# tspooner/rl_markets

Measured on NVIDIA H100. Metric: env steps/sec (batched LOBs), higher is better.
Workload: dtype f64

## Files before the change

rl_markets_b200/csrc/rlm_env.cuh:

```cuda
#pragma once
#include <cuda_runtime.h>
#include <math.h>
#include "rlm_types.h"

__constant__ DevParams P;

#define LLMIN ((long long)0x8000000000000000ull)
#ifdef RLM_ROLL_LEVELS
#define LEVEL_UNROLL _Pragma("unroll 1")
#else
#define LEVEL_UNROLL _Pragma("unroll")
#endif

__device__ __forceinline__ double pkey(double p) { return rint(p * 10000.0); }

__device__ __forceinline__ long long d2ll_x86(double d) {
  if (!(d >= -9223372036854775808.0 && d < 9223372036854775808.0)) return LLMIN;
  return (long long)d;
}

static_assert((RLM_MAX_BANDS & (RLM_MAX_BANDS - 1)) == 0, "the band search halves RLM_MAX_BANDS");
__device__ __noinline__ int to_ticks(double price, int* err, int* band_hint = nullptr) {
  const VenueD& V = P.venue;
  if (price < V.px[0]) { *err |= ERR_TICK_RANGE; return 0; }
// ... 271 lines not shown
}
__device__ __forceinline__ double win_back(const EnvHdr& e, const double* ring, int w) {
  int i = (e.w_count[w] == P.win_size[w]) ? e.w_head[w] : 0;
  return ring[P.win_off[w] + i];
}
__device__ __forceinline__ double win_std(const EnvHdr& e, int w) {
  double v = e.w_s[w] / (double)((unsigned long long)((long long)e.w_count[w] - 1));
  return v > 0 ? sqrt(v) : 0.0;
}

__device__ __noinline__ double get_reward(const EnvHdr& e) {
  double r = 0.0;
  long long ap = e.position < 0 ? -e.position : e.position;
  int abs_pos = (int)ap;
  switch (P.reward_measure) {
    case RLM_REWARD_NONE: break;
    case RLM_REWARD_PNL: r = e.pnl_step; break;
    case RLM_REWARD_PNL_DAMPED: r = e.pnl_step - (double)P.damping * fmax(0.0, e.momentum_pnl_step); break;
    case RLM_REWARD_SPREAD: r = e.pnl_step / e.w_mean[W_SPREAD]; break;
    case RLM_REWARD_NORMED:
      if (!(e.w_count[W_PNLUP] == P.win_size[W_PNLUP] && e.w_count[W_PNLDN] == P.win_size[W_PNLDN])) r = 0.0;
      else {
        double u = e.w_mean[W_PNLUP], d = e.w_mean[W_PNLDN];
        double su = win_std(e, W_PNLUP), sd = win_std(e, W_PNLDN);
        double numer = (u * sd - d * su), denom = (su + sd);
        if (isnan(numer) || isinf(numer)) numer = 0.0;
        if (isnan(denom) || isinf(denom)) denom = 0.0;
        r = (fabs(denom) < 1e-5) ? numer : (numer / denom);
      }
      break;
    case RLM_REWARD_LOVOL: r = (double)e.lo_vol_step; break;
    case RLM_REWARD_MM_LINEAR: r = (double)(-P.pos_weight * (float)abs_pos); r += (double)P.pnl_weight * e.pnl_step; break;
    case RLM_REWARD_MM_EXP:
      r = -pow(1.0 - exp((double)(P.pos_weight * (float)abs_pos)), 2.0); r += (double)P.pnl_weight * e.pnl_step; break;
    case RLM_REWARD_MM_DIV:
      if (e.pnl_step > 0) r = e.pnl_step / fmax(1.0, (double)abs_pos);
      else r = e.pnl_step;
      break;
  }
  return r * 100.0;
}

__device__ __noinline__ void clear_inventory(EnvHdr& e) {
  long long size = -e.position;
  Fill f; f.volume = 0; f.proxy = 0.0; f.value = 0.0;
  double mip = m_midprice(e);
  if (size > 0) f = side_walk<true>(e.side[0], mip, size);
  else if (size < 0) f = side_walk<false>(e.side[1], mip, size);
  e.position += f.volume;
  e.pnl_step += f.proxy;
  e.lo_vol_step += (int)(f.volume < 0 ? -f.volume : f.volume);
  e.ep_pnl += f.value;
  if (f.volume > 0) e.market_buys++;
  else if (f.volume < 0) e.market_sells++;
}

__device__ __noinline__ void place_orders(EnvHdr& e, int al, int bl) {
  e.ask_level = al; e.bid_level = bl;
  if (P.l2p_book) {
    e.ask_quote = to_price(to_ticks(e.side[0].px[0], &e.err, &e.tk_band) + al, &e.err);
    e.bid_quote = to_price(to_ticks(e.side[1].px[0], &e.err, &e.tk_band) - bl, &e.err);
  } else {
    double tp = e.tp_val, half_spd = fmax(0.0, e.w_mean[W_SPREAD] / 2.0);
    e.ask_quote = to_price(to_ticks(tp + (double)al * half_spd, &e.err, &e.tk_band), &e.err);
    e.bid_quote = to_price(to_ticks(tp - (double)bl * half_spd, &e.err, &e.tk_band), &e.err);
  }
  side_replace_order(e.side[0], e.ask_quote, P.order_size, &e.err);
  side_replace_order(e.side[1], e.bid_quote, P.order_size, &e.err);
}

__device__ __noinline__ void do_action(EnvHdr& e, int action) {
  int al, bl;
  switch (action) {
    case 0: al = 1; bl = 1; break;
    case 1: clear_inventory(e); al = e.ask_level; bl = e.bid_level; break;
    case 2: al = 2; bl = 2; break;
    case 3: al = 3; bl = 3; break;
    case 4: al = 0; bl = 2; break;
    case 5: al = 2; bl = 0; break;
    case 6: al = 1; bl = 4; break;
    case 7: al = 4; bl = 1; break;
    case 8: al = 5; bl = 5; break;
    default: return;
  }
  place_orders(e, al, bl);
}

__device__ __noinline__ void update_stats(EnvHdr& e) {
  e.ts_total++;
  bool has_ask = e.side[0].ord.live, has_bid = e.side[1].ord.live;
  if (has_ask) e.ts_ask++;
  if (has_bid) e.ts_bid++;
  if (has_ask && has_bid) e.ts_both++;
  if (e.position != 0) e.ts_pos++;
  if (e.position > 0) e.ts_long++;
  else if (e.position < 0) e.ts_short++;
}

__device__ __noinline__ void update_book_profiles(EnvHdr& e, const rlm_tick_msg& m) {
  e.last_date = e.date;
  e.date = m.date;
  e.time_ms = m.time_ms;
  side_apply_changes(e.side[0], m.ask_px, m.ask_vol, m, &e.err);
  side_apply_changes(e.side[1], m.bid_px, m.bid_vol, m, &e.err);
  if (e.side[0].has_last && e.side[1].has_last && !(pkey(e.side[0].last_px[0]) == 0.0) && !(pkey(e.side[1].last_px[0]) == 0.0)) {
    double mp = m_midprice(e);
    bool ok = (m_spread(e) >= 0.0) && (mp > 0.0) && (fabs(mp - m_last_midprice(e)) < mp);
    if (!ok) e.err |= ERR_INVALID_STATE;
  }
}

__device__ __noinline__ void next_state_tail(EnvHdr& e, const Fill& au, const Fill& bu, double* pushv) {
  Fill as = adverse_selection(e);
  e.pnl_step += au.proxy + bu.proxy + as.proxy;
  long long asabs = as.volume < 0 ? -as.volume : as.volume;
  e.lo_vol_step += (int)(bu.volume - au.volume + asabs);
  e.ep_pnl += au.value + bu.value + as.value;
  e.position += bu.volume + au.volume + as.volume;
  check_orders(e);
  double mid = m_midprice(e);
  long long mpt;
  if (mid == e.tk_px && mid > 0.0) mpt = e.tk_ticks;
  else { const int t = to_ticks(mid, &e.err, &e.tk_band); mpt = t; e.tk_px = mid; e.tk_ticks = t; }
  double mpm = mid - m_last_midprice(e), sp = m_spread(e);
  pushv[W_MID] = (double)mpt;
  pushv[W_VLT] = (double)mpt;
  pushv[W_VNUM] = e.side[0].obs_value + e.side[1].obs_value;
  pushv[W_VDEN] = (double)(e.side[0].obs_volume + e.side[1].obs_volume);
  pushv[W_SPREAD] = fmax(0.0, sp);
  pushv[W_TP] = P.tp_is_micro ? m_microprice(e) : mid;
  pushv[W_ASKTX] = (double)e.side[0].obs_volume;
  pushv[W_BIDTX] = (double)e.side[1].obs_volume;
  e.ewma_up = (P.ewma_alpha * fmax(0.0, mpm)) + ((1 - P.ewma_alpha) * e.ewma_up);
  e.ewma_dn = (P.ewma_alpha * fabs(fmin(0.0, mpm))) + ((1 - P.ewma_alpha) * e.ewma_dn);
  e.n_ticks++;
}

__device__ __forceinline__ void check_valid_state(EnvHdr& e) {
  if (e.side[0].has_last && e.side[1].has_last && !(pkey(e.side[0].last_px[0]) == 0.0) && !(pkey(e.side[1].last_px[0]) == 0.0)) {
    double mp = m_midprice(e);
    bool ok = (m_spread(e) >= 0.0) && (mp > 0.0) && (fabs(mp - m_last_midprice(e)) < mp);
    if (!ok) e.err |= ERR_INVALID_STATE;
  }
}

__device__ __noinline__ void next_state_scalar(EnvHdr& e, const rlm_tick_msg& m, double* pushv) {
  double mp = m_midprice(e);
  Fill au = side_apply_transactions<true>(e.side[0], m, mp, true);
  Fill bu = side_apply_transactions<false>(e.side[1], m, mp, true);
  update_book_profiles(e, m);
  next_state_tail(e, au, bu, pushv);
}

__device__ __noinline__ void next_state_warp(EnvHdr& e, const rlm_tick_msg& m, double* pushv, Fill* fills, int lane) {
  int* serr = (int*)(fills + 2);
  if (lane < 2) {
    const double mp = m_midprice(e);
    serr[lane] = 0;
    fills[lane] = (lane == 0) ? side_apply_transactions<true>(e.side[0], m, mp, true)
                              : side_apply_transactions<false>(e.side[1], m, mp, true);
  }
  __syncwarp();
  if (lane < 2) side_apply_changes(e.side[lane], lane == 0 ? m.ask_px : m.bid_px, lane == 0 ? m.ask_vol : m.bid_vol, m, &serr[lane]);
  __syncwarp();
  if (lane == 0) {
    e.last_date = e.date; e.date = m.date; e.time_ms = m.time_ms;
    e.err |= serr[0] | serr[1];
    check_valid_state(e);
    next_state_tail(e, fills[0], fills[1], pushv);
  }
}

__device__ __forceinline__ bool needs_multi(const EnvHdr& e, const rlm_tick_msg& m) { return (m.flags & 3) != 0 || e.tick_open != 0 || e.txn != 0; }
__device__ __forceinline__ void tick_tx_append(EnvHdr& e, const rlm_tick_msg& m) {
  for (int i = 0; i < m.n_tx && i < RLM_N_TX_MAX; ++i) {
    if (e.txn >= RLM_TX_CAP) { e.err |= ERR_BAD_PRICE; break; }
    e.tx_px[e.txn] = m.tx_px[i]; e.tx_vol[e.txn] = m.tx_vol[i]; e.txn++;
  }
}
__device__ __noinline__ bool update_book_profiles_multi(EnvHdr& e, const rlm_tick_msg& m, bool with_tx) {
  if (m.flags & RLM_TICK_TX_MORE) { if (with_tx && !e.tick_open) tick_tx_append(e, m); return false; }
  if (!e.tick_open) {
    if (with_tx) tick_tx_append(e, m); else e.txn = 0;
    side_stash(e.side[0]);
    side_stash(e.side[1]);
  }
  e.last_date = e.date;
  e.date = m.date;
  e.time_ms = m.time_ms;
  side_apply_row(e.side[0], m.ask_px, m.ask_vol, e.tx_px, e.tx_vol, e.txn, &e.err);
  side_apply_row(e.side[1], m.bid_px, m.bid_vol, e.tx_px, e.tx_vol, e.txn, &e.err);
  if (m.flags & RLM_TICK_PARTIAL) { e.tick_open = 1; return false; }
  e.tick_open = 0;
  e.txn = 0;
  return true;
}
__device__ __noinline__ bool next_state_multi(EnvHdr& e, const rlm_tick_msg& m, double* pushv) {
  if (m.flags & RLM_TICK_TX_MORE) { if (!e.tick_open) tick_tx_append(e, m); return false; }
  if (!e.tick_open) {
    tick_tx_append(e, m);
    const double mp = m_midprice(e);
    const Fill au = side_apply_transactions_n<true>(e.side[0], e.tx_px, e.tx_vol, e.txn, mp);
    const Fill bu = side_apply_transactions_n<false>(e.side[1], e.tx_px, e.tx_vol, e.txn, mp);
    e.tick_au.volume = au.volume; e.tick_au.proxy = au.proxy; e.tick_au.value = au.value;
    e.tick_bu.volume = bu.volume; e.tick_bu.proxy = bu.proxy; e.tick_bu.value = bu.value;
    side_stash(e.side[0]);
    side_stash(e.side[1]);
  }
  e.last_date = e.date;
  e.date = m.date;
  e.time_ms = m.time_ms;
  side_apply_row(e.side[0], m.ask_px, m.ask_vol, e.tx_px, e.tx_vol, e.txn, &e.err);
  side_apply_row(e.side[1], m.bid_px, m.bid_vol, e.tx_px, e.tx_vol, e.txn, &e.err);
  if (m.flags & RLM_TICK_PARTIAL) { e.tick_open = 1; return false; }
  e.tick_open = 0;
  e.txn = 0;
  check_valid_state(e);
  Fill au, bu;
  au.volume = e.tick_au.volume; au.proxy = e.tick_au.proxy; au.value = e.tick_au.value;
  bu.volume = e.tick_bu.volume; bu.proxy = e.tick_bu.proxy; bu.value = e.tick_bu.value;
  next_state_tail(e, au, bu, pushv);
  return true;
}

__device__ __forceinline__ double ulb_ref(double val, double lb, double ub) {
  const double m = (ub < val) ? ub : val;
  return (m < lb) ? lb : m;
}

__device__ __forceinline__ bool var_tick_args(const EnvHdr& e, const double* ring, int v, double& x0, double& x1) {
  switch (v) {
    case RLM_VAR_SPD: x0 = e.side[0].px[0]; x1 = e.side[1].px[0]; return true;
    case RLM_VAR_MPM: x0 = win_front(e, ring, W_MID); x1 = win_back(e, ring, W_MID); return true;
    case RLM_VAR_A_DIST: if (!e.side[0].ord.live) return false; x0 = e.side[0].ord.price; x1 = e.side[0].px[0]; return true;
    case RLM_VAR_B_DIST: if (!e.side[1].ord.live) return false; x0 = e.side[1].px[0]; x1 = e.side[1].ord.price; return true;
  }
  return false;
}
__device__ __forceinline__ double var_from_ticks(int v, int t0, int t1) {
  switch (v) {
    case RLM_VAR_SPD: return ulb_ref((double)(t0 - t1), 0.0, 20.0);
    case RLM_VAR_MPM: return ulb_ref((double)(t0 - t1), -10.0, 10.0);
  }
  return (double)t0 - (double)t1;
}

__device__ __noinline__ double get_variable(EnvHdr& e, const double* ring, int v) {
  switch (v) {
    case RLM_VAR_POS: return (double)e.position / (double)P.order_size;
    case RLM_VAR_SPD: {
      double d = (double)(to_ticks(e.side[0].px[0], &e.err, &e.tk_band) - to_ticks(e.side[1].px[0], &e.err, &e.tk_band));
      return ulb_ref(d, 0.0, 20.0);
    }
    case RLM_VAR_MPM: {
      double d = (double)(to_ticks(win_front(e, ring, W_MID), &e.err, &e.tk_band) - to_ticks(win_back(e, ring, W_MID), &e.err, &e.tk_band));
      return ulb_ref(d, -10.0, 10.0);
    }
    case RLM_VAR_IMB: {
      double v_a = (double)e.side[0].total_vol, v_b = (double)e.side[1].total_vol;
      return ((v_a + v_b) > 0 ? 5.0 * (v_b - v_a) / (v_b + v_a) : 0.0);
    }
    case RLM_VAR_SVL: {
      double q_a = e.w_sum[W_ASKTX], q_b = e.w_sum[W_BIDTX];
      return ((q_a + q_b) > 0 ? 5.0 * (q_b - q_a) / (q_a + q_b) : 0.0);
    }
    case RLM_VAR_VOL: return ulb_ref(5.0 * win_std(e, W_VLT), 0.0, 10.0);
    case RLM_VAR_RSI: {
      double u = e.ewma_up, d = e.ewma_dn;
      return (u + d) != 0.0 ? 5.0 * (u - d) / (u + d) : 0.0;
    }
    case RLM_VAR_VWAP: {
      double d = e.w_sum[W_VNUM] / e.w_sum[W_VDEN];
      return ulb_ref(d / e.w_mean[W_SPREAD], -10.0, 10.0);
    }
    case RLM_VAR_A_DIST:
      if (e.side[0].ord.live) return ((double)to_ticks(e.side[0].ord.price, &e.err, &e.tk_band) - (double)to_ticks(e.side[0].px[0], &e.err, &e.tk_band));
      else return -100.0;
    case RLM_VAR_A_QUEUE:
      if (e.side[0].ord.live) {
        float qp = (float)e.side[0].ord.q_head / fmaxf(1.0f, (float)e.side[0].ord.initial_queue);
        return 10.0 * (double)(long long)qp;
      } else return -1.0;
    case RLM_VAR_B_DIST:
      if (e.side[1].ord.live) return ((double)to_ticks(e.side[1].px[0], &e.err, &e.tk_band) - (double)to_ticks(e.side[1].ord.price, &e.err, &e.tk_band));
      else return -100.0;
    case RLM_VAR_B_QUEUE:
      if (e.side[1].ord.live) {
        float qp = (float)e.side[1].ord.q_head / fmaxf(1.0f, (float)e.side[1].ord.initial_queue);
        return 10.0 * (double)(long long)qp;
      } else return -1.0;
    case RLM_VAR_LAST_ACTION: return (double)e.last_action;
  }
  return 0.0;
}
```

rl_markets_b200/csrc/rlm_kernels.cu:

```cuda
#include <cuda_runtime.h>
#include <stdint.h>
#define RLM_TABLE_QUAL static __device__ const
#include "rlm_flow_tables.h"
#include "rlm_rndseq.h"
#include "rlm_agent.cuh"
#include <cstdio>
#include "rlm_kernels.h"
#define RLM_ENVT_CARVEOUT_DEFAULT 30
#define RLM_SMEM_CARVEOUT 88

#define SCR_Q 0
#define SCR_SS (SCR_Q + 8 * 2 * RLM_MAX_ACTIONS)
#define SCR_IDX (SCR_SS + 4 * SS_SLOTS)
#define SCR_VBUF (SCR_IDX + 4 * 3 * RLM_MAX_ACTIONS * 32)
#define AG_BYTES ((sizeof(AgentD) + 15) & ~(size_t)15)
size_t rlm_scratch_bytes(int is_double) {
  return ((size_t)SCR_VBUF + (size_t)(is_double ? 2 : 1) * RLM_MAX_ACTIONS * VROW * 8 + 15) & ~(size_t)15;
}
size_t rlm_agent_smem_bytes(int warps_per_cta, int scratch_bytes) {
  return (size_t)warps_per_cta * (AG_BYTES + (size_t)scratch_bytes);
}

#define PDL_PROLOGUE() do { asm volatile("griddepcontrol.launch_dependents;" ::: "memory"); asm volatile("griddepcontrol.wait;" ::: "memory"); } while (0)
static bool g_use_pdl = false;
void rlm_set_pdl(int on) { g_use_pdl = on != 0; }
template <typename... KArgs, typename... Args>
static cudaError_t launch_pdl(void (*kernel)(KArgs...), int grid, int block, size_t smem, cudaStream_t st, Args... args) {
  cudaLaunchConfig_t cfg = {};
  cfg.gridDim = dim3(grid); cfg.blockDim = dim3(block); cfg.dynamicSmemBytes = smem; cfg.stream = st;
  cudaLaunchAttribute at[1];
  at[0].id = cudaLaunchAttributeProgrammaticStreamSerialization;
  at[0].val.programmaticStreamSerializationAllowed = g_use_pdl ? 1 : 0;
  cfg.attrs = at; cfg.numAttrs = 1;
  return cudaLaunchKernelEx(&cfg, kernel, args...);
}

#ifdef RLM_TIMING
__device__ unsigned long long g_klog[256][8][2][2];
__device__ __forceinline__ unsigned long long gtime() { unsigned long long t; asm volatile("mov.u64 %0, %%globaltimer;" : "=l"(t)); return t; }
#define KLOG_BEGIN(kind) do { if (threadIdx.x == 0 && tslot < 256) atomicMin(&g_klog[tslot][D.sub_idx & 7][kind][0], gtime()); } while (0)
#define KLOG_END(kind) do { if (threadIdx.x == 0 && tslot < 256) atomicMax(&g_klog[tslot][D.sub_idx & 7][kind][1], gtime()); } while (0)
extern "C" int rlm_debug_klog(unsigned long long* out, int reset) {
  cudaDeviceSynchronize();
  if (out && cudaMemcpyFromSymbol(out, g_klog, sizeof(g_klog)) != cudaSuccess) return -1;
  if (reset) {
    static unsigned long long init[256][8][2][2];
    for (auto& a : init) for (auto& b : a) for (auto& c : b) { c[0] = ~0ull; c[1] = 0ull; }
    if (cudaMemcpyToSymbol(g_klog, init, sizeof(init)) != cudaSuccess) return -1;
  }
  return 0;
}
#else
#define KLOG_BEGIN(kind) do { } while (0)
#define KLOG_END(kind) do { } while (0)
#endif

cudaError_t rlm_upload_params(const DevParams* p) { return cudaMemcpyToSymbol(P, p, sizeof(DevParams)); }

__global__ void rlm_init_kernel(DevPtrs ptr, int mode) {
  int b = blockIdx.x * blockDim.x + threadIdx.x;
  if (b >= P.n_envs) return;
  EnvHdr* e = (EnvHdr*)(ptr.env + (size_t)b * P.env_stride);
  double* ring = (double*)((unsigned char*)e + sizeof(EnvHdr));
  if (mode == 0 || mode == 2) {
    AgentD keep;
    if (mode == 2) keep = e->ag;
    unsigned char* raw = (unsigned char*)e;
    for (int i = 0; i < P.env_stride; ++i) raw[i] = 0;
    for (int i = 0; i < P.ring_total; ++i) ring[i] = 0.0;
    e->tp_val = -1.0;
    if (mode == 2) e->ag = keep;
  }
  side_reset(e->side[0]);
  side_reset(e->side[1]);
  e->ask_quote = 0.0; e->bid_quote = 0.0;
  e->ep_reward = 0.0; e->ep_pnl = 0.0; e->ep_bandh = 0.0;
  e->market_buys = 0; e->market_sells = 0;
  e->ts_total = e->ts_ask = e->ts_bid = e->ts_both = e->ts_pos = e->ts_long = e->ts_short = 0;
  for (int w = 0; w < RLM_NWIN; ++w) { e->w_head[w] = 0; e->w_count[w] = 0; }
  e->last_date = 0; e->date = 0; e->time_ms = 0;
  e->phase = PH_PREOPEN;
  e->ag.ep_step = 0;
  if (mode == 1) {
    for (int i = 0; i < RLM_N_STATE_MAX + 3; ++i) e->ag.from_vars[i] = e->ag.prev_vars[i];
    e->ag.null_from = e->ag.prev_null;
  } else {
    e->ag.null_from = 1;
    e->ag.prev_null = 1;
  }
  e->ag.need_begin = 0;
  e->ag.kind = 0;
  rlm_flow_init(&e->flow, &P.flow, (uint64_t)(P.env_index0 + b));
  if (P.source == RLM_SOURCE_TAPE) ptr.tape_cur[b].x = ptr.tape_lo[b];
}

__global__ void rlm_seed_kernel(DevPtrs ptr, unsigned random_seed) {
  int b = blockIdx.x * blockDim.x + threadIdx.x;
  if (b >= P.n_envs) return;
  EnvHdr* e = (EnvHdr*)(ptr.env + (size_t)b * P.env_stride);
  unsigned seed = random_seed + (unsigned)(P.env_index0 + b);
  for (int g = 0; g < 2; ++g) {
    unsigned long long* x = g == 0 ? ptr.mt_pol : ptr.mt_agt;
    if (!x) continue;
    x += (size_t)b * 312;
    unsigned long long v = (unsigned long long)seed;
    x[0] = v;
    for (int i = 1; i < 312; ++i) { v = 6364136223846793005ull * (v ^ (v >> 62)) + (unsigned long long)i; x[i] = v; }
  }
  e->ag.mt_pol_idx = 312;
  e->ag.mt_agt_idx = 312;
  unsigned s = seed == 0 ? 1u : seed;
  e->ag.crand_r[0] = (int)s;
  for (int i = 1; i < 31; ++i) {
    long long hi = e->ag.crand_r[i - 1] / 127773, lo = e->ag.crand_r[i - 1] % 127773;
    long long word = 16807 * lo - 2836 * hi;
    if (word < 0) word += 2147483647;
    e->ag.crand_r[i] = (int)word;
  }
  e->ag.crand_f = 3; e->ag.crand_b = 0;
  for (int i = 0; i < 310; ++i) crand_next(e->ag);
}

__global__ void rlm_random_init_kernel(DevPtrs ptr, int n_policies) {
  int b = blockIdx.x * blockDim.x + threadIdx.x;
  if (b >= n_policies) return;
  EnvHdr* e = (EnvHdr*)(ptr.env + (size_t)b * P.env_stride);
  unsigned long long* x = ptr.mt_agt + (size_t)b * 312;
  double* th = ptr.theta + (size_t)b * P.memory_size;
  for (long long i = 0; i < P.memory_size; ++i) th[i] = 2.0 * mt_uniform_real(x, e->ag.mt_agt_idx) - 1.0;
  e->ag.n_occ = (int)P.memory_size;
  if (ptr.theta_b) {
    double* tb = ptr.theta_b + (size_t)b * P.memory_size;
    for (long long i = 0; i < P.memory_size; ++i) tb[i] = 2.0 * mt_uniform_real(x, e->ag.mt_agt_idx) - 1.0;
  }
}

__global__ void rlm_clear_traces_kernel(DevPtrs ptr) {
  int b = blockIdx.x * blockDim.x + threadIdx.x;
  if (b >= P.n_envs) return;
  EnvHdr* e = (EnvHdr*)(ptr.env + (size_t)b * P.env_stride);
  e->ag.n_traces = 0;
}

__global__ void rlm_gather_kernel(DevPtrs ptr, int what, void* out) {
  int b = blockIdx.x * blockDim.x + threadIdx.x;
  if (b >= P.n_envs) return;
  const EnvHdr* e = (const EnvHdr*)(ptr.env + (size_t)b * P.env_stride);
  if (what == 0) ((double*)out)[b] = e->ag.last_reward;
  else if (what == 1) ((int*)out)[b] = e->last_action;
  else if (what == 3) ((double*)out)[b] = e->ag.rho;
  else if (what == 4) ((int*)out)[b] = e->ag.n_occ;
  else
    for (int k = 0; k < P.n_state_vars; ++k) ((float*)out)[(size_t)b * P.n_state_vars + k] = e->ag.from_vars[k];
}

__global__ void rlm_count_nonzero_kernel(const double* theta, long long M, int* out) {
  const double* th = theta + (size_t)blockIdx.x * (size_t)M;
  int n = 0;
  for (long long i = threadIdx.x; i < M; i += blockDim.x) n += (__double_as_longlong(__ldcs(th + i)) != 0ll) ? 1 : 0;
  for (int o = 16; o > 0; o >>= 1) n += __shfl_xor_sync(FULL, n, o);
  __shared__ int part[8];
  if ((threadIdx.x & 31) == 0) part[threadIdx.x >> 5] = n;
  __syncthreads();
  if (threadIdx.x == 0) { int t = 0; for (int w = 0; w < (int)(blockDim.x >> 5); ++w) t += part[w]; out[blockIdx.x] = t; }
}
cudaError_t rlm_launch_count_nonzero(const double* theta, long long M, int n_policies, int* out, cudaStream_t st) {
  rlm_count_nonzero_kernel<<<n_policies, 256, 0, st>>>(theta, M, out);
  return cudaGetLastError();
}

__device__ __noinline__ void fill_record(rlm_step_record* r, const EnvHdr& e, const AgentD& ag, unsigned long long thash,
                                         const float* vars) {
  r->step = ag.ep_step; r->action = ag.cur_action; r->time_ms = e.time_ms; r->terminal = is_terminal(e) ? 1 : 0;
  r->position = e.position; r->ask_quote = e.ask_quote; r->bid_quote = e.bid_quote;
  r->ask_level = e.ask_level; r->bid_level = e.bid_level;
  r->reward = ag.last_reward; r->pnl_step = e.pnl_step;
  r->ep_pnl = e.ep_pnl; r->ep_reward = e.ep_reward; r->ep_bandh = e.ep_bandh;
  r->midprice = m_midprice(e); r->spread = m_spread(e); r->bandh_step = e.agg_mpm;
  for (int s = 0; s < 2; ++s) {
    rlm_order_rec& o = s == 0 ? r->ask : r->bid;
    const OrderD& d = e.side[s].ord;
    o.exists = d.live ? 1 : 0; o.pad = 0;
    o.price = d.live ? d.price : 0.0; o.q_head = d.live ? d.q_head : 0; o.q_tail = d.live ? d.q_tail : 0;
    o.executed = d.live ? (d.size - ord_remaining(d)) : 0;
  }
  r->ask_transactions = e.side[0].n_transacted; r->bid_transactions = e.side[1].n_transacted;
  r->market_buys = e.market_buys; r->market_sells = e.market_sells;
  r->lo_vol_step = e.lo_vol_step;
  r->n_state = P.n_state_vars;
  for (int i = 0; i < RLM_N_STATE_MAX + 1; ++i) r->state[i] = (i < P.n_state_vars) ? vars[i] : 0.0f;
  r->delta = ag.last_delta;
  r->n_traces = ag.n_traces; r->pad = 0;
  r->trace_hash = thash;
}

__device__ __noinline__ int begin_select(EnvHdr& e, unsigned long long* mt_pol, const DynParams& D) {
  if (is_terminal(e)) {
    clear_inventory(e);
    e.phase = PH_DONE;
    return -1;
  }
  return policy_action(e.ag, e.ag.q_from, e.ag.qb_from, mt_pol, D);
}
__device__ __noinline__ void begin_apply(EnvHdr& e, int a) {
  e.ag.cur_action = a;
  e.last_action = a;
  e.lo_vol_step = 0;
// ... 389 lines not shown
  const unsigned m = __ballot_sync(FULL, ready >= 0);
  if (m) {
    const int leader = __ffs(m) - 1;
    int base = 0;
    if (lane == leader) base = atomicAdd(&ptr.ready_count[tslot], __popc(m));
    base = __shfl_sync(FULL, base, leader);
    if (ready >= 0) ptr.ready[base + __popc(m & ((1u << lane) - 1u))] = b;
  }
  if (!only_begin) KLOG_END(0);
  const unsigned tm = __ballot_sync(FULL, ticked != 0);
  unsigned em = errs;
  for (int o = 16; o > 0; o >>= 1) em |= __shfl_xor_sync(FULL, em, o);
  if (lane == 0) {
    if (tm) atomicAdd(&ptr.counters[0], (unsigned long long)__popc(tm));
    if (em) atomicOr(&ptr.counters[4], (unsigned long long)em);
  }
}

#define ENVW_WARPS 8
#define ENVW_WARPS_DEFAULT 8
__host__ __device__ inline size_t envw_hdr_bytes() { return (sizeof(EnvHdr) + 15) & ~(size_t)15; }
__host__ __device__ inline size_t envw_warp_bytes() { return envw_hdr_bytes() + 128 + 8 * 2 * RLM_NWIN + 128; }
struct EnvWarp {
  EnvHdr* e; rlm_tick_msg* msg; double* pushv; double* oldv; int* flag; unsigned* r12; Fill* fills;
};
__device__ __forceinline__ EnvWarp envw_carve(unsigned char* wbase) {
  EnvWarp w;
  const size_t hb = envw_hdr_bytes();
  w.e = (EnvHdr*)wbase;
  w.msg = (rlm_tick_msg*)(wbase + hb);
  w.pushv = (double*)(wbase + hb + 128);
  w.oldv = w.pushv + RLM_NWIN;
  w.flag = (int*)(w.oldv + RLM_NWIN);
  w.r12 = (unsigned*)(w.flag + 4);
  w.fills = (Fill*)(w.r12 + 12);
  return w;
}
__device__ __forceinline__ void envw_stage_in(EnvHdr* dst_e, const EnvHdr* g, int lane) {
  const int4* src = (const int4*)g;
  int4* dst = (int4*)dst_e;
  const int n16 = (int)(envw_hdr_bytes() / 16);
  static_assert(sizeof(EnvHdr) <= 4 * 32 * 16, "four 16-byte loads per lane cover the env header");
  int4 t[4];
#pragma unroll
  for (int k = 0; k < 4; ++k) { const int i = lane + 32 * k; if (i < n16) t[k] = src[i]; }
#pragma unroll
  for (int k = 0; k < 4; ++k) { const int i = lane + 32 * k; if (i < n16) dst[i] = t[k]; }
}
__device__ __forceinline__ unsigned envw_stage_in_tape(EnvHdr* dst_e, const EnvHdr* g, const DevPtrs& ptr, int env, int lane, bool l2_next,
                                                       int2& tc) {
  tc = ptr.tape_cur[env];
  const int4* src = (const int4*)g;
  int4* dst = (int4*)dst_e;
  const int n16 = (int)(envw_hdr_bytes() / 16);
  int4 t[4];
#pragma unroll
  for (int k = 0; k < 4; ++k) { const int i = lane + 32 * k; if (i < n16) t[k] = src[i]; }
  unsigned word = 0;
  if (tc.x < tc.y) word = __ldg((const unsigned*)(ptr.tape + tc.x) + lane);
  if (l2_next && lane == 0 && tc.x + 1 < tc.y) asm volatile("prefetch.global.L2 [%0];" ::"l"(ptr.tape + tc.x + 1));
#pragma unroll
  for (int k = 0; k < 4; ++k) { const int i = lane + 32 * k; if (i < n16) dst[i] = t[k]; }
  return word;
}
__device__ __forceinline__ void envw_stage_out(EnvHdr* g, const EnvHdr* src_e, int lane) {
  int4* dst = (int4*)g;
  const int4* src = (const int4*)src_e;
  for (int i = lane; i < (int)(envw_hdr_bytes() / 16); i += 32) dst[i] = src[i];
}

template <bool TAPE = false>
__device__ __forceinline__ int envw_tick(const EnvWarp& w, double* ring, const DevPtrs& ptr, const DynParams& D, int env, int stream_pos,
                                         int stream_ticks, int lane, unsigned& ticked, unsigned tape_word = 0) {
  EnvHdr& e = *w.e;
  rlm_tick_msg& msg = *w.msg;
  double* pushv = w.pushv;
  double* oldv = w.oldv;
  int ready = -1;
  bool have = true;
  if (TAPE) {
    if (stream_pos >= stream_ticks) have = false;
    else ((unsigned*)&msg)[lane] = tape_word;
  } else if (P.source == RLM_SOURCE_GENERATOR) {
    flow_next_warp(&e.flow, &msg, w.r12, lane);
  } else {
    if (stream_pos >= stream_ticks) { if (lane == 0) e.err |= ERR_STREAM_UNDERRUN; have = false; }
    else ((unsigned*)&msg)[lane] = __ldg((const unsigned*)(ptr.stream + ((size_t)stream_pos * P.n_envs + env)) + lane);
  }
  if (lane < RLM_NWIN) oldv[lane] = window_peek(e, ring, lane);
  __syncwarp();
  const int phase = e.phase;
  const bool multi = have && needs_multi(e, msg);
  int complete = 1;
  if (multi && phase != PH_PREOPEN) {
    if (lane == 0) {
      if (phase == PH_RUN) e.pnl_step = 0.0;
      complete = next_state_multi(e, msg, pushv) ? 1 : 0;
    }
    complete = __shfl_sync(FULL, complete, 0);
  }
  if (have && phase == PH_PREOPEN) {
    if (lane == 0) {
      if (multi) {
        if (update_book_profiles_multi(e, msg, false) && market_is_open(e)) e.phase = PH_WARMUP;
      } else {
        msg.n_tx = 0;
        update_book_profiles(e, msg);
        if (market_is_open(e)) e.phase = PH_WARMUP;
      }
    }
  } else if (have && complete) {
    ticked += 1;
    if (!multi) {
      if (lane == 0 && phase == PH_RUN) e.pnl_step = 0.0;
      __syncwarp();
      next_state_warp(e, msg, pushv, w.fills, lane);
    }
    __syncwarp();
    if (lane < 8) window_push(e, ring, lane, pushv[lane], oldv[lane]);
    __syncwarp();
    if (lane == 0) {
      int r = -1;
      e.tp_val = e.w_mean[W_TP];
      if (phase == PH_WARMUP) {
        bool full = true;
        for (int k = 0; k < 8; ++k) full = full && (e.w_count[k] == P.win_size[k]);
        if (full) {
          place_orders(e, 1, 1);
          e.phase = PH_RUN;
          e.ag.kind = 1;
          r = 1;
        }
      } else {
        double mpm = m_midprice(e) - m_last_midprice(e);
        e.pnl_step += (double)e.position * mpm;
        e.momentum_pnl_step += (double)e.position * mpm;
        e.agg_r += get_reward(e);
        e.agg_pnl += e.pnl_step;
        e.agg_mpm += mpm;
        if (!(!is_terminal(e) && fabs(e.agg_mpm) < 1e-5)) {
          e.pnl_step = e.agg_pnl;
          pushv[W_PNLUP] = fmax(0.0, e.pnl_step);
          pushv[W_PNLDN] = fabs(fmin(0.0, e.pnl_step));
          e.ep_reward += e.agg_r;
          e.ep_bandh += e.agg_mpm;
          r = 0;
        }
      }
      *w.flag = r;
    }
    __syncwarp();
    ready = *w.flag;
    if (ready == 0) {
      if (lane == W_PNLUP || lane == W_PNLDN) window_push(e, ring, lane, pushv[lane], oldv[lane]);
      __syncwarp();
      {
        const bool has = lane < P.n_state_vars;
        const int var = has ? P.state_vars[lane] : -1;
        double x0 = 0.0, x1 = 0.0;
        const bool two = has && var_tick_args(e, ring, var, x0, x1);
        int t0 = 0, t1 = 0, lerr = 0, hint = e.tk_band;
        if (two) { t0 = to_ticks(x0, &lerr, &hint); t1 = to_ticks(x1, &lerr, &hint); }
        if (lerr) atomicOr(&e.err, lerr);
        if (has) e.ag.to_vars[lane] = (float)(two ? var_from_ticks(var, t0, t1) : get_variable(e, ring, var));
      }
      if (lane == 31) { e.ag.last_reward = get_reward(e); e.ag.kind = 0; }
      if (D.env_hash && !D.backtest && !P.shared_policy && P.algorithm < RLM_ALGO_R_LEARN) {
        __syncwarp();
        const LnSums h = ln_hash(rlm_rndseq_table, e.ag.to_vars, false, lane);
        unsigned long long* hs = ptr.hsum + (size_t)env * 96;
        hs[lane] = h.s[0]; hs[32 + lane] = h.s[1]; hs[64 + lane] = h.s[2];
        const double* th_a = ptr.theta + (size_t)env * (size_t)P.memory_size;
        const double* th_b = ptr.theta_b ? ptr.theta_b + (size_t)env * (size_t)P.memory_size : nullptr;
#pragma unroll 1
        for (int g = 0; g < 3; ++g) {
#pragma unroll
          for (int a = 0; a < RLM_MAX_ACTIONS; ++a) {
            if (a < P.n_actions) {
              const int f = mod_m(h.s[g] + P.rg[g][a]);
              asm volatile("prefetch.global.L2 [%0];" ::"l"(th_a + f));
              if (th_b) asm volatile("prefetch.global.L2 [%0];" ::"l"(th_b + f));
            }
          }
        }
        if (lane == 0) e.ag.hs_valid = 1;
      }
    } else if (ready == 1 && D.backtest) {
      if (lane < P.n_state_vars) e.ag.to_vars[lane] = (float)get_variable(e, ring, P.state_vars[lane]);
    }
  }
  __syncwarp();
  return ready;
}

template <bool TAPE>
__global__ void __launch_bounds__(ENVW_WARPS * 32) rlm_env_kernel_w(DevPtrs ptr, DynParams D, int tslot, int only_begin) {
  PDL_PROLOGUE();
  extern __shared__ __align__(16) unsigned char smem[];
  const int tid = threadIdx.x, lane = tid & 31, warp = tid >> 5;
  const int env = D.env0 + blockIdx.x * (blockDim.x >> 5) + warp;
  if (!only_begin) KLOG_BEGIN(0);
  if (env >= (D.n_sub > 0 ? D.env0 + D.n_sub : P.n_envs)) return;
  const EnvWarp w = envw_carve(smem + (size_t)warp * envw_warp_bytes());
  EnvHdr& e = *w.e;
  EnvHdr* g = (EnvHdr*)(ptr.env + (size_t)env * P.env_stride);
  double* ring = (double*)((unsigned char*)g + sizeof(EnvHdr));
  if (only_begin && !g->ag.need_begin) return;
  const bool tape = TAPE && !only_begin;
  int2 tc = make_int2(0, 0);
  unsigned tape_word = 0;
  if (tape) tape_word = envw_stage_in_tape(&e, g, ptr, env, lane, D.tape_l2 != 0, tc);
  else envw_stage_in(&e, g, lane);
  __syncwarp();
  if (e.phase == PH_DONE) return;
  if (D.hold && env_on_hold(e)) return;
  int ready = -1;
  unsigned ticked = 0;
  bool starved = false;
  if (e.ag.need_begin) begin_step_warp(e, ptr.mt_pol + (size_t)env * 312, D, w.flag, lane);
  if (!only_begin && e.phase != PH_DONE) {
    if (tape) {
      starved = tc.x >= tc.y;
      if (!starved) {
        ready = envw_tick<true>(w, ring, ptr, D, env, tc.x, tc.y, lane, ticked, tape_word);
        if (lane == 0) ptr.tape_cur[env].x = tc.x + 1;
      }
    } else if (D.ctl_stream) {
      const int4 rc4 = __ldg((const int4*)ptr.runctl);
      DevPtrs pt = ptr;
      pt.stream = (const rlm_tick_msg*)__ldg((const unsigned long long*)ptr.runctl + 2);
      ready = envw_tick(w, ring, pt, D, env, rc4.z + tslot, rc4.w, lane, ticked);
    } else {
      ready = envw_tick(w, ring, ptr, D, env, D.stream_off + tslot, D.stream_ticks, lane, ticked);
    }
  }
  __syncwarp();
  envw_stage_out(g, &e, lane);
  if (!only_begin) KLOG_END(0);
  if (lane == 0) {
    if (ready >= 0) ptr.ready[atomicAdd(&ptr.ready_count[tslot], 1)] = env;
    if (D.hold && ready < 0 && e.phase != PH_DONE && !starved) atomicAdd(&ptr.counters[5], 1ull);
    if (ticked) atomicAdd(&ptr.counters[0], 1ull);
    const unsigned errs = (unsigned)(e.err | e.ag.err);
    if (errs) atomicOr(&ptr.counters[4], (unsigned long long)errs);
  }
}

template <bool TAPE>
__global__ void __launch_bounds__(ENVW_WARPS * 32, 4) rlm_env_round_kernel(DevPtrs ptr, DynParams D, int tslot) {
  PDL_PROLOGUE();
  extern __shared__ __align__(16) unsigned char smem[];
  const int tid = threadIdx.x, lane = tid & 31, warp = tid >> 5;
  const int env = D.env0 + blockIdx.x * (blockDim.x >> 5) + warp;
  KLOG_BEGIN(0);
  if (env >= (D.n_sub > 0 ? D.env0 + D.n_sub : P.n_envs)) return;
  int* live_count = ptr.ready_count + RLM_LIVE_OFF;
  if (tslot > 0 && __ldcg(live_count + tslot - 1) == 0) return;
  const int4 rc4 = __ldg((const int4*)ptr.runctl);
  const RunCtl rc = {rc4.x, rc4.y, rc4.z, rc4.w, nullptr, 0};
  DevPtrs pt = ptr;
  pt.stream = (const rlm_tick_msg*)__ldg((const unsigned long long*)ptr.runctl + 2);
  const EnvWarp w = envw_carve(smem + (size_t)warp * envw_warp_bytes());
  EnvHdr& e = *w.e;
  EnvHdr* g = (EnvHdr*)(ptr.env + (size_t)env * P.env_stride);
  double* ring = (double*)((unsigned char*)g + sizeof(EnvHdr));
  const bool tape = TAPE;
  int2 tc = make_int2(0, 0);
  unsigned tape_word = 0;
  if (tape) tape_word = envw_stage_in_tape(&e, g, ptr, env, lane, false, tc);
  else envw_stage_in(&e, g, lane);
  __syncwarp();
  if (e.phase == PH_DONE) return;
  int pos = e.run_id == rc.run_id ? e.run_pos : 0;
  if (pos >= rc.n_ticks && !e.ag.need_begin) return;
  int ready = -1;
  unsigned ticked = 0;
  const int cap = D.round_cap > 0 ? D.round_cap : 0x7fffffff;
  int n_run = 0;
  bool starved = false;
#pragma unroll 1
  for (;;) {
    if (e.ag.need_begin) begin_step_warp(e, ptr.mt_pol + (size_t)env * 312, D, w.flag, lane);
    if (e.phase == PH_DONE || pos >= rc.n_ticks || n_run >= cap) break;
    if (tape) {
      if (tc.x >= tc.y) { starved = true; break; }
      const unsigned word = tape_word;
      if (tc.x + 1 < tc.y) tape_word = __ldg((const unsigned*)(ptr.tape + tc.x + 1) + lane);
      ready = envw_tick<true>(w, ring, pt, D, env, tc.x, tc.y, lane, ticked, word);
      ++tc.x;
    } else {
      ready = envw_tick(w, ring, pt, D, env, rc.stream_off + pos, rc.stream_ticks, lane, ticked);
    }
    ++pos; ++n_run;
    if (ready >= 0) break;
  }
  if (lane == 0) {
    e.run_id = rc.run_id; e.run_pos = pos;
    if (tape) {
      ptr.tape_cur[env].x = tc.x;
      if (D.tape_l2 && tc.x < tc.y) asm volatile("prefetch.global.L2 [%0];" ::"l"(ptr.tape + tc.x));
    }
  }
  __syncwarp();
  envw_stage_out(g, &e, lane);
  KLOG_END(0);
  if (lane == 0) {
    if (ready >= 0) ptr.ready[atomicAdd(&ptr.ready_count[tslot], 1)] = env;
    if (ready >= 0 || (e.phase != PH_DONE && pos < rc.n_ticks && !starved)) atomicAdd(&live_count[tslot], 1);
    if (ticked) atomicAdd(&ptr.counters[0], (unsigned long long)ticked);
    const unsigned errs = (unsigned)(e.err | e.ag.err);
    if (errs) atomicOr(&ptr.counters[4], (unsigned long long)errs);
  }
}
__global__ void rlm_runctl_kernel(RunCtl* dst, RunCtl v) { *dst = v; }

__device__ __forceinline__ void emit_record(const DevPtrs& ptr, const EnvHdr* g, int env, const AgentD& ag, const double* theta_a,
                                         const float* vars, int lane) {
  const int* tf = ptr.trace_f + (size_t)env * P.trace_cap;
  const float* te = ptr.trace_e + (size_t)env * P.trace_cap;
  unsigned long long h = trace_hash(tf, te, theta_a, ag.n_traces, lane);
  if (lane == 0) {
    int c = ptr.record_count[env];
    if (c < P.record_cap) {
      EnvHdr tmp;
      const int4* src = (const int4*)g;
      int4* dst = (int4*)&tmp;
      for (int i = 0; i < (int)(sizeof(EnvHdr) / 16); ++i) dst[i] = __ldcg(src + i);
      fill_record(&ptr.records[(size_t)env * P.record_cap + c], tmp, ag, h, vars);
    }
    ptr.record_count[env] = c + 1;
  }
}

__device__ __noinline__ void emit_record_ool(const DevPtrs& ptr, const EnvHdr* g, int env, const AgentD& ag, const double* theta_a,
                                             const float* vars, int lane) {
  emit_record(ptr, g, env, ag, theta_a, vars, lane);
}
__device__ __noinline__ void emit_record_res(const DevPtrs& ptr, const EnvHdr* e, int env, const AgentD& ag, const double* theta_a,
                                             const float* vars, int lane) {
  const int* tf = ptr.trace_f + (size_t)env * P.trace_cap;
  const float* te = ptr.trace_e + (size_t)env * P.trace_cap;
  const unsigned long long h = trace_hash(tf, te, theta_a, ag.n_traces, lane);
  if (lane == 0) {
    const int c = ptr.record_count[env];
    if (c < P.record_cap) fill_record(&ptr.records[(size_t)env * P.record_cap + c], *e, ag, h, vars);
    ptr.record_count[env] = c + 1;
  }
}

__device__ __forceinline__ void backtest_advance(const DevPtrs& ptr, const EnvHdr* g, int env, AgentD& ag, const double* theta_a,
                                                 int kind, double qa, double qb, unsigned long long base0, int lane,
                                                 unsigned long long& steps_done) {
  if (kind == 0) {
    if (lane == 0) ag.last_delta = 0.0;
    __syncwarp();
    if (env < P.record_envs) emit_record_ool(ptr, g, env, ag, theta_a, ag.from_vars, lane);
    __syncwarp();
  }
  if (lane < P.n_actions) { ag.q_from[lane] = qa; ag.qb_from[lane] = qb; }
  if (lane < RLM_N_STATE_MAX + 3) ag.from_vars[lane] = ag.to_vars[lane];
  ag.from_base0[lane] = mod_m(base0);
  if (lane == 0) {
    ag.null_from = 0; ag.need_begin = 1;
    if (kind == 0) { ag.n_steps++; ag.ep_step++; } else ag.kind = 2;
  }
  if (kind == 0) steps_done++;
}

__device__ __noinline__ void td_decision(AgentD& ag, const double* q_pre_a, const double* q_pre_b, unsigned long long* mt_pol,
                                         unsigned long long* mt_agt, const DynParams& D, double* out) {
  ASSUME_SHARED(&ag); ASSUME_SHARED(q_pre_a); ASSUME_SHARED(q_pre_b); ASSUME_SHARED(out); ASSUME_GLOBAL(mt_pol);
  const int action = ag.cur_action;
  const double reward = ag.last_reward;
  const double F_term = P.gamma * 0.0 - 0.0;
  float rate = P.gl;
  double delta;
  int table = 0;
  if (P.algorithm == RLM_ALGO_SARSA) {
    double Q1 = ag.q_from[action];
    int a2 = policy_action(ag, q_pre_a, q_pre_b, mt_pol, D);
    double Q2 = q_pre_a[a2];
    delta = reward + F_term + P.gamma * Q2 - Q1;
  } else if (P.algorithm == RLM_ALGO_Q_LEARN) {
    int amax = argmax_ties_fast(ag, ag.q_from);
    if (action != amax) rate = 0.0f;
    double Q = ag.q_from[action];
    int am2 = argmax_ties_fast(ag, q_pre_a);
    delta = reward + F_term + P.gamma * q_pre_a[am2] - Q;
  } else if (P.algorithm == RLM_ALGO_DOUBLE_Q_LEARN) {
    int amax = argmax_ties_fast(ag, ag.q_from);
    if (action != amax) rate = 0.0f;
    if (mt_uniform_real(mt_agt, ag.mt_agt_idx) > 0.5) {
      double Qa = ag.q_from[action];
      int am2 = argmax_ties_fast(ag, q_pre_a);
      delta = reward + F_term + P.gamma * q_pre_b[am2] - Qa;
      table = 0;
    } else {
      double Qb = ag.qb_from[action];
      int am2 = argmax_ties_fast(ag, q_pre_b);
      delta = reward + F_term + P.gamma * q_pre_a[am2] - Qb;
      table = 1;
    }
  } else if (P.algorithm == RLM_ALGO_R_LEARN) {
    int amax = argmax_ties_fast(ag, ag.q_from);
    if (action != amax) rate = 0.0f;
    double Q = ag.q_from[action];
    double mQ = q_pre_a[argmax_ties_fast(ag, q_pre_a)];
    delta = reward - ag.rho + mQ - Q;
    out[3] = Q; out[4] = mQ;
  } else if (P.algorithm == RLM_ALGO_ONLINE_R_LEARN) {
    double Q = ag.q_from[action];
    double gQ = q_pre_a[policy_action(ag, q_pre_a, q_pre_b, mt_pol, D)];
    delta = reward - ag.rho + gQ - Q;
    out[3] = Q; out[4] = gQ;
  } else {
    int amax = argmax_ties_fast(ag, ag.q_from);
    if (action != amax) rate = 0.0f;
    double Q, mQ;
    if (mt_uniform_real(mt_agt, ag.mt_agt_idx) > 0.5) {
      Q = ag.q_from[action];
      mQ = q_pre_b[argmax_ties_fast(ag, q_pre_a)];
      table = 0;
    } else {
      Q = ag.qb_from[action];
      mQ = q_pre_a[argmax_ties_fast(ag, q_pre_b)];
      table = 1;
    }
    delta = reward - ag.rho + mQ - Q;
    out[3] = Q; out[4] = mQ;
  }
  ag.last_delta = delta;
  out[0] = (double)rate;
  out[1] = (D.alpha * delta) * (1.0 / (double)RLM_N_TILINGS);
  out[2] = (double)table;
}

__device__ __noinline__ void td_rho(AgentD& ag, const double* q_post_a, const double* q_post_b, const DynParams& D, const double* dec) {
  const double Q = dec[3];
  double boot = dec[4];
  const double nQ = Q + D.alpha * ag.last_delta;
  double best;
  if (P.algorithm == RLM_ALGO_DOUBLE_R_LEARN) {
    best = -1.7976931348623157e308;
    for (int i = 0; i < P.n_actions; i++) {
      double val = (q_post_a[i] + q_post_b[i]) / 2.0;
      if (val > best) best = val;
    }
    boot = best;
  } else {
    best = q_post_a[argmax_ties(ag, q_post_a)];
  }
  if (nQ - best < 1e-7) ag.rho += P.beta * (ag.last_reward - ag.rho + boot - nQ);
}

#ifdef RLM_TIMING
__device__ long long g_phase_clk[4096 * 16];
__device__ unsigned g_phase_sm[4096];
#define PH(i) do { if (tid == 0 && idx < 4096) { g_phase_clk[idx * 16 + (i)] = clock64(); if ((i) == 0) { unsigned s_; asm volatile("mov.u32 %0, %%smid;" : "=r"(s_)); g_phase_sm[idx] = s_; } } } while (0)
extern "C" int rlm_debug_read_phases(long long* clk, unsigned* sm) {
  cudaDeviceSynchronize();
  if (cudaMemcpyFromSymbol(clk, g_phase_clk, sizeof(long long) * 4096 * 16) != cudaSuccess) return -1;
  if (cudaMemcpyFromSymbol(sm, g_phase_sm, sizeof(unsigned) * 4096) != cudaSuccess) return -1;
  long long tp[8];
  if (cudaMemcpyFromSymbol(tp, g_tp_clk, sizeof(tp)) == cudaSuccess)
    printf("slowest trace_pass so far: %lld cycles = set build %lld + decay loop %lld + set() %lld; n=%lld decay=%lld\n", tp[0], tp[1], tp[2], tp[3],
// ... 980 lines not shown
```

Baseline: 12.28 million.

## Spread book-level updates across warp lanes in next_state_warp

Replaces the two-lane side_apply_changes call with a per-level parallel update in which each of 2*RLM_DEPTH lanes copies one price/volume level and checks validity, combined through a warp ballot. Two lanes then finish the per-side totals and order updates. It also adds a non-templated side_apply_transactions_lane so both sides run the same code path instead of diverging templates. Separately it adds optional clock64 phase timing instrumentation under RLM_TIMING. The risk is semantic drift from the original side_apply_changes, for example in error flags, tick-key checks or the total_vol accumulation, which now adds onto the old total_vol.

```diff
diff --git a/rl_markets_b200/csrc/rlm_env.cuh b/rl_markets_b200/csrc/rlm_env.cuh
--- a/rl_markets_b200/csrc/rlm_env.cuh
+++ b/rl_markets_b200/csrc/rlm_env.cuh
@@ -447,20 +447,74 @@
   next_state_tail(e, au, bu, pushv);
 }
 
+__device__ __noinline__ Fill side_apply_transactions_lane(SideD& s, const rlm_tick_msg& m, double ref, bool is_ask) {
+  const int n = m.n_tx;
+  s.obs_value = 0.0;
+  s.obs_volume = 0;
+  Fill f; f.volume = 0; f.proxy = 0.0; f.value = 0.0;
+  OrderD& o = s.ord;
+  for (int k = 0; k < n; ++k) {
+    const int i = is_ask ? k : n - 1 - k;
+    const double tp = (double)m.tx_px[i];
+    if (is_ask ? (tp < ref) : (tp > ref)) continue;
+    long long vol = m.tx_vol[i];
+    s.obs_value += tp * (double)vol;
+    s.obs_volume += vol;
+    while (o.live && (is_ask ? (o.price <= tp) : (o.price >= tp))) {
+      long long rem0 = ord_remaining(o);
+      vol = ord_do_transaction(o, vol);
+      long long exec = rem0 - ord_remaining(o);
+      f.volume += is_ask ? -exec : exec;
+      f.proxy += (is_ask ? (o.price - ref) : (ref - o.price)) * (double)exec;
+      const double pv = o.price * (double)exec;
+      f.value += is_ask ? pv : -pv;
+      if (ord_is_executed(o)) { o.live = 0; s.n_transacted++; }
+      if (vol <= 0) break;
+    }
+  }
+  return f;
+}
+
 __device__ __noinline__ void next_state_warp(EnvHdr& e, const rlm_tick_msg& m, double* pushv, Fill* fills, int lane) {
-  int* serr = (int*)(fills + 2);
   if (lane < 2) {
     const double mp = m_midprice(e);
-    serr[lane] = 0;
-    fills[lane] = (lane == 0) ? side_apply_transactions<true>(e.side[0], m, mp, true)
-                              : side_apply_transactions<false>(e.side[1], m, mp, true);
+    fills[lane] = side_apply_transactions_lane(e.side[lane], m, mp, lane == 0);
   }
   __syncwarp();
-  if (lane < 2) side_apply_changes(e.side[lane], lane == 0 ? m.ask_px : m.bid_px, lane == 0 ? m.ask_vol : m.bid_vol, m, &serr[lane]);
+  bool bad = false;
+  if (lane < 2 * RLM_DEPTH) {
+    const int sd = lane >= RLM_DEPTH ? 1 : 0, l = lane - sd * RLM_DEPTH;
+    SideD& s = e.side[sd];
+    const double p = (double)(sd == 0 ? m.ask_px : m.bid_px)[l];
+    const int v = (sd == 0 ? m.ask_vol : m.bid_vol)[l];
+    s.last_px[l] = s.px[l]; s.last_vol[l] = s.vol[l];
+    bad = p <= 0.0 || v <= 0;
+    s.px[l] = p; s.vol[l] = v;
+  }
+  const bool any_bad = __ballot_sync(0xffffffffu, bad) != 0;
+  __syncwarp();
+  if (lane < 2) {
+    SideD& s = e.side[lane];
+    const int* vol = lane == 0 ? m.ask_vol : m.bid_vol;
+    s.has_last = s.has_cur;
+    s.last_total_vol = s.total_vol;
+    long long tv = s.total_vol;
+#pragma unroll
+    for (int l = 0; l < RLM_DEPTH; ++l) tv += vol[l];
+    s.total_vol = tv;
+    s.has_cur = 1;
+    if (s.ord.live) {
+      long long t = 0;
+      double k = pkey(s.ord.price);
+      for (int i = 0; i < m.n_tx; ++i)
+        if (pkey((double)m.tx_px[i]) == k) t = m.tx_vol[i];
+      side_update_order(s, t);
+    }
+  }
   __syncwarp();
   if (lane == 0) {
     e.last_date = e.date; e.date = m.date; e.time_ms = m.time_ms;
-    e.err |= serr[0] | serr[1];
+    if (any_bad) e.err |= ERR_BAD_PRICE;
     check_valid_state(e);
     next_state_tail(e, fills[0], fills[1], pushv);
   }
diff --git a/rl_markets_b200/csrc/rlm_kernels.cu b/rl_markets_b200/csrc/rlm_kernels.cu
--- a/rl_markets_b200/csrc/rlm_kernels.cu
+++ b/rl_markets_b200/csrc/rlm_kernels.cu
@@ -53,6 +53,27 @@
 #else
 #define KLOG_BEGIN(kind) do { } while (0)
 #define KLOG_END(kind) do { } while (0)
+#endif
+
+#ifdef RLM_TIMING
+enum { TK_STAGE_IN, TK_BEGIN, TK_TICK, TK_STEP_END, TK_WRITE_BACK, TK_N_TICKS, TK_FLAGS, TK_TOTAL, TK_NS0, TK_NS1, TK_TAKEN = 15 };
+__device__ long long g_tick_clk[16384 * 16];
+__device__ __forceinline__ long long tk_clock() { return clock64(); }
+extern "C" int rlm_debug_read_tick_phases(long long* out, int reset) {
+  cudaDeviceSynchronize();
+  if (out && cudaMemcpyFromSymbol(out, g_tick_clk, sizeof(g_tick_clk)) != cudaSuccess) return -1;
+  if (reset) {
+    void* p = nullptr;
+    if (cudaGetSymbolAddress(&p, g_tick_clk) != cudaSuccess || cudaMemset(p, 0, sizeof(g_tick_clk)) != cudaSuccess) return -1;
+  }
+  return cudaDeviceSynchronize() == cudaSuccess ? 0 : -1;
+}
+#define TK_ON 1
+#define TK_MARK(k) do { const long long t_ = clock64(); tk[k] += t_ - tk_t; tk_t = t_; } while (0)
+#else
+#define TK_ON 0
+#define TK_MARK(k) do { } while (0)
+__device__ __forceinline__ long long tk_clock() { return 0; }
 #endif
 
 cudaError_t rlm_upload_params(const DevParams* p) { return cudaMemcpyToSymbol(P, p, sizeof(DevParams)); }
@@ -748,6 +769,7 @@
     __syncwarp();
     ready = *w.flag;
     if (ready == 0) {
+      const long long tk0 = tk_clock();
       if (lane == W_PNLUP || lane == W_PNLDN) window_push(e, ring, lane, pushv[lane], oldv[lane]);
       __syncwarp();
       {
@@ -781,6 +803,7 @@
         }
         if (lane == 0) e.ag.hs_valid = 1;
       }
+      if (TK_ON && lane == 0) w.flag[2] = (int)(tk_clock() - tk0);
     } else if (ready == 1 && D.backtest) {
       if (lane < P.n_state_vars) e.ag.to_vars[lane] = (float)get_variable(e, ring, P.state_vars[lane]);
     }
@@ -849,6 +872,12 @@
   const int tid = threadIdx.x, lane = tid & 31, warp = tid >> 5;
   const int env = D.env0 + blockIdx.x * (blockDim.x >> 5) + warp;
   KLOG_BEGIN(0);
+#ifdef RLM_TIMING
+  const unsigned long long tk_ns0 = gtime();
+  long long tk_t = clock64(), tk[TK_WRITE_BACK + 1] = {0, 0, 0, 0, 0};
+  const long long tk_c0 = tk_t;
+  int tk_flags = 0;
+#endif
   if (env >= (D.n_sub > 0 ? D.env0 + D.n_sub : P.n_envs)) return;
   int* live_count = ptr.ready_count + RLM_LIVE_OFF;
   if (tslot > 0 && __ldcg(live_count + tslot - 1) == 0) return;
@@ -874,9 +903,16 @@
   const int cap = D.round_cap > 0 ? D.round_cap : 0x7fffffff;
   int n_run = 0;
   bool starved = false;
+  TK_MARK(TK_STAGE_IN);
 #pragma unroll 1
   for (;;) {
-    if (e.ag.need_begin) begin_step_warp(e, ptr.mt_pol + (size_t)env * 312, D, w.flag, lane);
+    if (e.ag.need_begin) {
+      begin_step_warp(e, ptr.mt_pol + (size_t)env * 312, D, w.flag, lane);
+#ifdef RLM_TIMING
+      tk_flags |= 1;
+#endif
+    }
+    TK_MARK(TK_BEGIN);
     if (e.phase == PH_DONE || pos >= rc.n_ticks || n_run >= cap) break;
     if (tape) {
       if (tc.x >= tc.y) { starved = true; break; }
@@ -887,6 +923,11 @@
     } else {
       ready = envw_tick(w, ring, pt, D, env, rc.stream_off + pos, rc.stream_ticks, lane, ticked);
     }
+    TK_MARK(TK_TICK);
+#ifdef RLM_TIMING
+    if (ready == 0) { tk[TK_TICK] -= w.flag[2]; tk[TK_STEP_END] += w.flag[2]; }
+    if (ready >= 0) tk_flags |= 2;
+#endif
     ++pos; ++n_run;
     if (ready >= 0) break;
   }
@@ -907,6 +948,15 @@
     const unsigned errs = (unsigned)(e.err | e.ag.err);
     if (errs) atomicOr(&ptr.counters[4], (unsigned long long)errs);
   }
+#ifdef RLM_TIMING
+  TK_MARK(TK_WRITE_BACK);
+  long long* tr = g_tick_clk + (size_t)env * 16;
+  if (lane == 0 && env < 16384 && tr[TK_TAKEN] == 0) {
+    for (int k = 0; k <= TK_WRITE_BACK; ++k) tr[k] = tk[k];
+    tr[TK_N_TICKS] = n_run; tr[TK_FLAGS] = tk_flags; tr[TK_TOTAL] = tk_t - tk_c0;
+    tr[TK_NS0] = (long long)tk_ns0; tr[TK_NS1] = (long long)gtime(); tr[TK_TAKEN] = 1;
+  }
+#endif
 }
 __global__ void rlm_runctl_kernel(RunCtl* dst, RunCtl v) { *dst = v; }
 
```

New measurement: 12.45 million (median of 6 runs). 1.01x the previous value.
